# ningyu1991/InclusiveGAN

Measured on AMD Instinct MI355X. Metric: training img/sec (whole node), CelebA 128x128 StyleGAN2+IMLE, higher is better.
Workload: dtype f32-equivalent (3x3 convs: 2-piece fp16 split, operands to <= 1 ulp of fp32, scales per pixel / per channel: no per-tensor window; fp32 sums)

## Files before the change

### inclusivegan_amd/csrc/conv2d_mfma.hip

```cpp
#include "igan_common.h"
#include <cmath>
#include <cstdlib>
#include <type_traits>

namespace {

typedef float f32x16 __attribute__((ext_vector_type(16)));

constexpr int BK = 32;
#ifndef IGAN_SPLIT
#define IGAN_SPLIT 8
#endif
constexpr int LDK = BK + 4;

struct ConvArgs {
    const float* x;
    const float* w;
    float* y;
    float* out;
    const float* in_scale;
    const float* out_scale;
    int N, H, W, Cin;
    int OH, OW, Cout;
    int KH, KW;
// ... 2483 lines not shown
            const f16x8 b0 = __builtin_bit_cast(f16x8, tr8(S, fB[0], fB[1]));
            const f16x8 b1 = __builtin_bit_cast(f16x8, tr8(S + 4096, fB[0], fB[1]));
#pragma unroll
            for (int tm = 0; tm < TM; tm++) {
                a0[tm] = __builtin_bit_cast(f16x8, tr8(S, fA[tm][0], fA[tm][1]));
                a1[tm] = __builtin_bit_cast(f16x8, tr8(S + 4096, fA[tm][0], fA[tm][1]));
            }
            dma_prep(nst);
            f32x16 t;
            __builtin_amdgcn_sched_barrier(0);
            t = __builtin_amdgcn_mfma_f32_32x32x16_f16(a0[0], b0, zero, 0, 0, 0);
            u[0] = __builtin_amdgcn_mfma_f32_32x32x16_f16(a0[0], b1, u[0], 0, 0, 0);
            u[1] = __builtin_amdgcn_mfma_f32_32x32x16_f16(a0[1], b1, u[1], 0, 0, 0);
            __builtin_amdgcn_sched_barrier(0);
            dma_piece(0); dma_piece(1);
            acc[0] += t;
            __builtin_amdgcn_sched_barrier(0);
            t = __builtin_amdgcn_mfma_f32_32x32x16_f16(a0[1], b0, zero, 0, 0, 0);
            u[0] = __builtin_amdgcn_mfma_f32_32x32x16_f16(a1[0], b0, u[0], 0, 0, 0);
            u[1] = __builtin_amdgcn_mfma_f32_32x32x16_f16(a1[1], b0, u[1], 0, 0, 0);
            acc[1] += t;
            st = (st + 1 == P_NSTAGE) ? 0 : st + 1;
        }
        const float* xinv = reinterpret_cast<const float*>(reinterpret_cast<const unsigned char*>(a.xp) + (size_t)a.N * a.H * a.W * a.Cin * 4);
        const float* dyinv = reinterpret_cast<const float*>(reinterpret_cast<const unsigned char*>(a.dyp) + (size_t)a.N * a.OH * a.OW * a.Cout * 4);
        const int co_ = n0 + wn * 32 + l31;
        const float inv_b = (co_ < a.Cout) ? dyinv[co_] : 0.0f;
#pragma unroll
        for (int tm = 0; tm < TM; tm++)
#pragma unroll
            for (int q = 0; q < 4; q++) {
                const int ci = m0 + wm * 64 + tm * 32 + 8 * q + 4 * h;
                const float4 ia = (ci < a.Cin) ? *reinterpret_cast<const float4*>(xinv + ci) : f4zero();
                acc[tm][4 * q + 0] = ((acc[tm][4 * q + 0] + u[tm][4 * q + 0] * (1.0f / 2048.0f)) * ia.x) * inv_b;
                acc[tm][4 * q + 1] = ((acc[tm][4 * q + 1] + u[tm][4 * q + 1] * (1.0f / 2048.0f)) * ia.y) * inv_b;
                acc[tm][4 * q + 2] = ((acc[tm][4 * q + 2] + u[tm][4 * q + 2] * (1.0f / 2048.0f)) * ia.z) * inv_b;
                acc[tm][4 * q + 3] = ((acc[tm][4 * q + 3] + u[tm][4 * q + 3] * (1.0f / 2048.0f)) * ia.w) * inv_b;
            }
    } else
    for (int c = c_begin; c < c_end; c++) {
        asm volatile("s_waitcnt vmcnt(3)\n\ts_barrier" ::: "memory");
        const int nst = st >= 1 ? st - 1 : P_NSTAGE - 1;
        const unsigned char* S = smem + st * STAGE;
        bf16x8 af[TM][3], bfr[3];
#pragma unroll
        for (int q = 0; q < 3; q++) {
            bfr[q] = tr8(S + q * 4096, fB[0], fB[1]);
#pragma unroll
            for (int tm = 0; tm < TM; tm++) af[tm][q] = tr8(S + q * 4096, fA[tm][0], fA[tm][1]);
        }
        dma_prep(nst);
        f32x16 t[TM];
        __builtin_amdgcn_sched_barrier(0);
#pragma unroll
        for (int tm = 0; tm < TM; tm++) t[tm] = __builtin_amdgcn_mfma_f32_32x32x16_bf16(af[tm][0], bfr[0], zero, 0, 0, 0);
        int g = 0;
#pragma unroll
        for (int o = 1; o < 3; o++)
#pragma unroll
            for (int i = 0; i <= o; i++) {
                if (g == 2) { __builtin_amdgcn_sched_barrier(0); dma_piece(0); dma_piece(1); dma_piece(2); __builtin_amdgcn_sched_barrier(0); }
#pragma unroll
                for (int tm = 0; tm < TM; tm++) t[tm] = __builtin_amdgcn_mfma_f32_32x32x16_bf16(af[tm][i], bfr[o - i], t[tm], 0, 0, 0);
                ++g;
            }
#pragma unroll
        for (int tm = 0; tm < TM; tm++) acc[tm] += t[tm];
        st = (st + 1 == P_NSTAGE) ? 0 : st + 1;
    }
    drain_lds_dma();
    const size_t wsize = (size_t)a.KH * a.KW * a.Cin * a.Cout;
    float* out = a.out + (a.splits > 1 ? (size_t)split * wsize : (size_t)0) + (size_t)tap * a.Cin * a.Cout;
    const float alpha = (a.splits == 1) ? a.alpha : 1.0f;
    const int co = n0 + wn * 32 + l31;
#pragma unroll
    for (int tm = 0; tm < TM; tm++)
#pragma unroll
        for (int r = 0; r < 16; r++) {
            const int ci = m0 + wm * 64 + tm * 32 + (r & 3) + 8 * (r >> 2) + 4 * h;
            if (ci < a.Cin && co < a.Cout) out[(size_t)ci * a.Cout + co] = acc[tm][r] * alpha;
        }
}

__global__ __launch_bounds__(256) void plain_reduce_kernel(const float* ws, float* y, int total, int splits, float alpha) {
    for (int i = blockIdx.x * blockDim.x + threadIdx.x; i < total; i += gridDim.x * blockDim.x) {
        float s0 = 0.f, s1 = 0.f, s2 = 0.f, s3 = 0.f;
        int k = 0;
        for (; k + 4 <= splits; k += 4) {
            const float a0 = ws[(size_t)k * total + i], a1 = ws[(size_t)(k + 1) * total + i];
            const float a2 = ws[(size_t)(k + 2) * total + i], a3 = ws[(size_t)(k + 3) * total + i];
            s0 += a0; s1 += a1; s2 += a2; s3 += a3;
        }
        for (; k < splits; k++) s0 += ws[(size_t)k * total + i];
        y[i] = ((s0 + s1) + (s2 + s3)) * alpha;
    }
}

struct FwdTile { int BM, BN; };

FwdTile pick_fwd_tile(int Mmax, int Cout) {
    FwdTile t;
    t.BN = (Cout > 64) ? 128 : (Cout > 32 ? 64 : 32);
    t.BM = (Mmax <= 32 && t.BN == 128) ? 32 : 128;
    return t;
}

int fwd_geometry_check(const igan_conv2d_params* p) {
    IGAN_REQUIRE(p->x && p->w && p->y, "conv2d: null buffer");
    IGAN_REQUIRE(p->N >= 1 && p->H >= 1 && p->W >= 1 && p->Cin >= 1, "conv2d: input dims must be positive");
    IGAN_REQUIRE(p->OH >= 1 && p->OW >= 1 && p->Cout >= 1, "conv2d: output dims must be positive");
    IGAN_REQUIRE(p->KH >= 1 && p->KW >= 1, "conv2d: kernel must be at least 1x1");
    IGAN_REQUIRE(p->stride >= 1 && p->up >= 1, "conv2d: stride and up must be at least 1");
    IGAN_REQUIRE(p->stride == 1 || p->up == 1, "conv2d: at most one of stride, up may exceed 1");
    if (!(p->up == 1 || p->up == 2)) return igan::fail(IGAN_ERR_UNSUPPORTED, "conv2d: up must be 1 or 2 (got %d)", p->up);
    IGAN_REQUIRE((long long)p->N * p->H * p->W * p->Cin * 4 <= 0x7FFFFFF0LL, "conv2d: input too large (2 GiB per operand)");
    IGAN_REQUIRE((long long)p->N * p->OH * p->OW * p->Cout <= INT32_MAX, "conv2d: output too large");
    IGAN_REQUIRE((long long)p->KH * p->KW * p->Cin * p->Cout * 4 <= 0x7FFFFFF0LL, "conv2d: filter too large (2 GiB per operand)");
    IGAN_REQUIRE(p->act >= 0 && p->act <= 3, "conv2d: fused epilogue act must be 0 (none), 1 linear, 2 relu or 3 lrelu");
    IGAN_REQUIRE(p->act == 0 || p->act_gain > 0.0f, "conv2d: fused epilogue gain must be positive");
    IGAN_REQUIRE(p->noise == nullptr || (p->act != 0 && p->noise_strength != nullptr), "conv2d: noise needs the fused epilogue (act != 0) and a strength scalar");
    return IGAN_OK;
}

bool eight_waves(const char* env) {
    const char* v = getenv(env);
    return !(v && atoi(v) == 0);
}

bool is_small_dense(const igan_conv2d_params* p) {
    return p->H == 1 && p->W == 1 && p->OH == 1 && p->OW == 1 && p->KH == 1 && p->KW == 1 && p->stride == 1 && p->up == 1 &&
           p->pad_y == 0 && p->pad_x == 0 && !p->in_scale && !p->out_scale && p->act == 0 &&
           igan::dense_small_ok(p->N, p->Cin, p->Cout, p->x, p->w, p->w_transposed != 0);
}
bool is_small_dense_wgrad(const igan_conv2d_wgrad_params* p) {
    return p->H == 1 && p->W == 1 && p->OH == 1 && p->OW == 1 && p->KH == 1 && p->KW == 1 && p->stride == 1 && p->up == 1 &&
           p->pad_y == 0 && p->pad_x == 0 && !p->in_scale && !p->out_scale &&
           igan::dense_small_wgrad_ok(p->N, p->Cout, p->dy, p->dw);
}

void fwd_counts(const igan_conv2d_params* p, int& Mmax, int& chunks_max, int& nclass) {
    const int up = p->up;
    nclass = up * up;
    const int QH = (p->OH + up - 1) / up, QW = (p->OW + up - 1) / up;
    Mmax = p->N * QH * QW;
    const int cpt = (p->Cin + BK - 1) / BK;
    chunks_max = ((p->KH + up - 1) / up) * ((p->KW + up - 1) / up) * cpt;
}

template <int BM, int BN, int WM, int WN, bool WT, bool VEC>
void launch_fwd2(hipStream_t stream, const ConvArgs& a, dim3 grid) {
    if (a.in_scale) hipLaunchKernelGGL((conv_fwd_kernel<BM, BN, WM, WN, WT, VEC, true>), grid, dim3(WM * WN * 64), 0, stream, a);
    else hipLaunchKernelGGL((conv_fwd_kernel<BM, BN, WM, WN, WT, VEC, false>), grid, dim3(WM * WN * 64), 0, stream, a);
}

template <int BM, int BN, int WM, int WN>
void launch_fwd(hipStream_t stream, const ConvArgs& a, dim3 grid, bool wt, bool vec) {
    if (wt) {
        if (vec) launch_fwd2<BM, BN, WM, WN, true, true>(stream, a, grid);
        else launch_fwd2<BM, BN, WM, WN, true, false>(stream, a, grid);
    } else {
        if (vec) launch_fwd2<BM, BN, WM, WN, false, true>(stream, a, grid);
        else launch_fwd2<BM, BN, WM, WN, false, false>(stream, a, grid);
    }
}

}
// ... 10 lines not shown
        (void)hipGetLastError();
        cus = n;
    }
    return cus;
}

struct TileList { int nx, ny, T, rem; };
TileList tile_list(const igan_conv2d_params* p, const FwdTile& t, int Mmax, int nclass) {
    TileList l;
    l.nx = igan::ceil_div(Mmax, t.BM);
    l.ny = igan::ceil_div(p->Cout, t.BN);
    l.T = l.nx * l.ny * nclass;
    l.rem = l.T % device_cus();
    return l;
}


bool use_dma_kernel(const igan_conv2d_params* p, const FwdTile& t, bool walk) {
    static const bool dma = !(getenv("IGAN_CONV_DMA") && atoi(getenv("IGAN_CONV_DMA")) == 0);
    if (!dma || t.BM != 128 || t.BN != 128 || !walk || !eight_waves("IGAN_CONV_8WAVE")) return false;
    if ((long long)p->N * p->OH * p->OW >= (1LL << 24)) return false;
    if (p->in_scale) {
        const int up = p->up;
        for (int c = 0; c < up * up; c++) {
            const int qh = (p->OH - c / up + up - 1) / up, qw = (p->OW - c % up + up - 1) / up;
            if (qh <= 0 || qw <= 0) continue;
            const int samples = 127 / (qh * qw) + 2;
            if ((long long)std::min(samples, p->N) * p->Cin > 2048) return false;
        }
    }
    return true;
}

bool walk_ok(const igan_conv2d_params* p) {
    static const bool walk = !(getenv("IGAN_CONV_WALK") && atoi(getenv("IGAN_CONV_WALK")) == 0);
    const bool wt = p->w_transposed != 0;
    const bool vecA = (p->Cin % 4 == 0) && (((uintptr_t)p->x & 15) == 0);
    const bool vecS = (p->Cin % 4 == 0) && (((uintptr_t)p->in_scale & 15) == 0);
    const bool vecB = ((wt ? p->Cin : p->Cout) % 4 == 0) && (((uintptr_t)p->w & 15) == 0);
    return walk && vecA && vecB && (p->in_scale == nullptr || vecS) && (p->Cin % BK == 0);
}

int planes_mode() {
    static const int mode = [] { const char* v = getenv("IGAN_CONV_PLANES"); const int m = v ? atoi(v) : 2; return m == 0 ? 0 : (m == 1 ? 1 : 2); }();
    return mode;
}
bool planes_enabled() { return planes_mode() != 0; }

int ilog2(int v) { int l = 0; while ((1 << l) < v) ++l; return l; }
bool pow2(int v) { return v > 0 && (v & (v - 1)) == 0; }

void launch_piece_image(hipStream_t stream, const float* x, const float* scale, unsigned short* out, int P_, int HW, int C) {
    const int cpp = C / PK, total = P_ * cpp;
    hipLaunchKernelGGL(to_planes_kernel, dim3(igan::ceil_div(total, 256)), dim3(256), 0, stream, x, scale, out, total, cpp, C, HW);
}
void launch_row_image(hipStream_t stream, const float* x, const float* scale, unsigned short* out, int P_, int HW, int C, float* colmax) {
    const int cpp = C / PK, total = P_ * cpp;
    float* rowinv = reinterpret_cast<float*>(reinterpret_cast<unsigned char*>(out) + (size_t)P_ * C * 4);
    const int nchunks = igan::ceil_div(total, 256);
    const int grid = colmax ? std::min(nchunks, H_COLBLOCKS) : nchunks;
    hipLaunchKernelGGL(rows_f16_kernel, dim3(grid), dim3(256), 0, stream, x, scale, out, rowinv, colmax, total, cpp, ilog2(cpp), C, HW);
}
void launch_colmax_only(hipStream_t stream, const float* x, const float* scale, float* colmax, int P_, int HW, int C) {
    const int C4 = C / 4, ppi = 256 / C4;
    const int blocks = std::min(H_COLBLOCKS, igan::ceil_div(P_, ppi));
    hipLaunchKernelGGL(cols_amax_kernel, dim3(blocks), dim3(256), 0, stream, x, scale, colmax + 4, P_, C4, ilog2(C4), HW, colmax);
}
void launch_col_image(hipStream_t stream, const float* x, const float* scale, unsigned short* out, int P_, int HW, int C, const float* colmax) {
    const int cpp = C / PK, total = P_ * cpp, C4 = C / 4;
    float* inv = reinterpret_cast<float*>(reinterpret_cast<unsigned char*>(out) + (size_t)P_ * C * 4);
    float* sc = inv + C;
    float* partial = sc + C;
    const int ppi = 256 / C4;
    const int blocks = std::min(H_COLBLOCKS, igan::ceil_div(P_, ppi));
    if (colmax == nullptr) {
        hipLaunchKernelGGL(cols_amax_kernel, dim3(blocks), dim3(256), 0, stream, x, scale, partial, P_, C4, ilog2(C4), HW, (float*)nullptr);
        hipLaunchKernelGGL(cols_finalize_kernel, dim3(igan::ceil_div(C, 8)), dim3(256), 0, stream, (const float*)partial, inv, sc, blocks, C, (const float*)nullptr);
    } else
        hipLaunchKernelGGL(cols_finalize_kernel, dim3(igan::ceil_div(C, 8)), dim3(256), 0, stream, colmax + 4, inv, sc, 0, C, colmax);
    hipLaunchKernelGGL(cols_f16_kernel, dim3(igan::ceil_div(total, 256)), dim3(256), 0, stream, x, scale, out, (const float*)sc, total, cpp, C, HW);
}
bool f16_tap_outer() { static const int v = getenv("IGAN_F16_TAP_OUTER") ? atoi(getenv("IGAN_F16_TAP_OUTER")) : 1; return v != 0; }
bool f16_w4() { static const int v = getenv("IGAN_F16_W4") ? atoi(getenv("IGAN_F16_W4")) : 1; return v != 0; }
void launch_filter_image(hipStream_t stream, const float* w, unsigned short* wp, bool wt, int taps, int KW_, int Nn, int K) {
    const int wtotal = taps * Nn * (K / PK);
    if (planes_mode() == 2) {
        float* inv = reinterpret_cast<float*>(reinterpret_cast<unsigned char*>(wp) + (size_t)taps * Nn * K * 4);
        float* partial = inv + Nn;
        if (wt) {
            hipLaunchKernelGGL((filter_amax_kernel<true>), dim3(igan::ceil_div(taps * Nn, 4)), dim3(256), 0, stream, w, partial, taps, Nn, K);
            hipLaunchKernelGGL((filter_planes_f16_kernel<true>), dim3(igan::ceil_div(wtotal, 256)), dim3(256), 0, stream, w, wp, inv, (const float*)partial, taps, taps, KW_, Nn, K);
        } else {
            hipLaunchKernelGGL((filter_amax_kernel<false>), dim3(taps * H_KSK, igan::ceil_div(Nn, 64)), dim3(256), 0, stream, w, partial, taps, Nn, K);
            hipLaunchKernelGGL((filter_planes_f16_kernel<false>), dim3(igan::ceil_div(wtotal, 256)), dim3(256), 0, stream, w, wp, inv, (const float*)partial, taps * H_KSK, taps, KW_, Nn, K);
        }
    } else {
        if (wt) hipLaunchKernelGGL((filter_planes_kernel<true>), dim3(igan::ceil_div(wtotal, 256)), dim3(256), 0, stream, w, wp, taps, KW_, Nn, K);
        else hipLaunchKernelGGL((filter_planes_kernel<false>), dim3(igan::ceil_div(wtotal, 256)), dim3(256), 0, stream, w, wp, taps, KW_, Nn, K);
    }
}

bool planes_shape_ok(const igan_conv2d_params* p, const FwdTile& t, int Mmax) {
    if (!planes_enabled() || t.BM != 128 || t.BN != 128 || p->Cin % BK != 0) return false;
    static const int min_rows = getenv("IGAN_PLANES_MIN_ROWS") ? atoi(getenv("IGAN_PLANES_MIN_ROWS")) : 1024;
    if (p->KH * p->KW == 1 || (long long)p->KH * p->KW * p->Cin < 1152 || Mmax < min_rows) return false;
    if ((long long)p->N * p->OH * p->OW >= (1LL << 24)) return false;
    if ((long long)p->N * p->H * p->W * p->Cin * 6 >= 0x7FFFFF00LL || (long long)p->KH * p->KW * p->Cin * p->Cout * 6 >= 0x7FFFFF00LL) return false;
    if (planes_mode() == 2 && (!pow2(p->Cin / PK) || p->Cin / PK > 64 || p->KH * p->KW > 9 || p->Cout % 4 != 0)) return false;
#ifdef IGAN_DIAGNOSTIC
    {
        static const int only_cin = getenv("IGAN_PLANES_ONLY_CIN") ? atoi(getenv("IGAN_PLANES_ONLY_CIN")) : 0;
        static const int no_act = getenv("IGAN_PLANES_NO_ACT") ? atoi(getenv("IGAN_PLANES_NO_ACT")) : 0;
        static const int no_scale = getenv("IGAN_PLANES_NO_SCALE") ? atoi(getenv("IGAN_PLANES_NO_SCALE")) : 0;
        static const int kind = getenv("IGAN_PLANES_KIND") ? atoi(getenv("IGAN_PLANES_KIND")) : 0;
        static const int wt = getenv("IGAN_PLANES_WT") ? atoi(getenv("IGAN_PLANES_WT")) : 0;
        if (only_cin && p->Cin != only_cin) return false;
        if ((no_act == 1 && p->act != 0) || (no_act == 2 && p->act == 0)) return false;
        if ((no_scale == 1 && p->in_scale != nullptr) || (no_scale == 2 && p->in_scale == nullptr)) return false;
        if ((kind == 1 && (p->stride != 1 || p->up != 1)) || (kind == 2 && p->stride != 2) || (kind == 3 && p->up != 2)) return false;
        if ((wt == 1 && p->w_transposed) || (wt == 2 && !p->w_transposed)) return false;
    }
#endif
    return true;
}
bool use_planes_kernel(const igan_conv2d_params* p, const FwdTile& t, int Mmax) {
    if (!planes_shape_ok(p, t, Mmax) || (((uintptr_t)p->x | (uintptr_t)p->w | (uintptr_t)p->in_scale | (uintptr_t)p->x_pieces) & 15) != 0) return false;
    if (planes_mode() == 2 && (((uintptr_t)p->y | (uintptr_t)p->out_scale | (uintptr_t)p->bias) & 15) != 0) return false;
    return true;
}
size_t planes_x_floats(const igan_conv2d_params* p) {
    if (planes_mode() == 2) return rows_part_bytes((size_t)p->N * p->H * p->W, (size_t)p->Cin) / 4;
    return (size_t)p->N * p->H * p->W * p->Cin * 6 / 4;
}
size_t planes_w_floats(const igan_conv2d_params* p) {
    if (planes_mode() == 2) return filter_part_bytes((size_t)p->KH * p->KW, (size_t)p->Cout, (size_t)p->Cin) / 4;
    return (size_t)p->KH * p->KW * p->Cin * p->Cout * 6 / 4;
}

}

static unsigned long long* g_conv_diag = nullptr;
extern "C" void igan_debug_set_conv_diag(unsigned long long* p) { g_conv_diag = p; }

static int conv2d_plan_tiles(const igan_conv2d_params* p, int* splits, int* sliced_tiles, size_t* workspace_floats);

extern "C" int igan_conv2d_plan(const igan_conv2d_params* p, int* splits, int* sliced_tiles, size_t* workspace_floats) {
    IGAN_REQUIRE(p && splits && sliced_tiles && workspace_floats, "conv2d_plan: null argument");
    if (int rc = fwd_geometry_check(p)) return rc;
    *splits = 1;
    *sliced_tiles = 0;
    *workspace_floats = 0;
    if (is_small_dense(p) || igan::thin_conv_kind(p)) return IGAN_OK;
    if (int rc = conv2d_plan_tiles(p, splits, sliced_tiles, workspace_floats)) return rc;
    int Mmax, chunks_max, nclass;
    fwd_counts(p, Mmax, chunks_max, nclass);
    if (planes_shape_ok(p, pick_fwd_tile(Mmax, p->Cout), Mmax))
        *workspace_floats += planes_x_floats(p) + planes_w_floats(p);
    return IGAN_OK;
}

static int conv2d_plan_tiles(const igan_conv2d_params* p, int* splits, int* sliced_tiles, size_t* workspace_floats) {
    int Mmax, chunks_max, nclass;
    fwd_counts(p, Mmax, chunks_max, nclass);
    const FwdTile t = pick_fwd_tile(Mmax, p->Cout);
    const TileList l = tile_list(p, t, Mmax, nclass);
    {
// ... 248 lines not shown
    WgTile t;
    t.BM = (Cin > 32) ? 128 : 32;
    t.BN = (Cout > 32) ? 128 : 32;
    if (t.BM == 32 && t.BN == 32) t.BN = 128;
    return t;
}

int wgrad_splits(const igan_conv2d_wgrad_params* p) {
    const WgTile t = pick_wg_tile(p->Cin, p->Cout);
    const long long tiles = (long long)igan::ceil_div(p->Cin, t.BM) * igan::ceil_div(p->Cout, t.BN) * p->KH * p->KW;
    const int up = p->up;
    const long long kpix = (long long)p->N * ((p->OH + up - 1) / up) * ((p->OW + up - 1) / up);
    const int chunks = (int)((kpix + BK - 1) / BK);
    const int max_by_work = std::max(1, chunks / 4);
    int s;
    if (tiles >= 512) s = 1;
    else {
        s = (int)(512 / tiles);
        if (s > max_by_work) s = max_by_work;
        else if (chunks / s > 96 && 1024 / tiles <= max_by_work) s = (int)(1024 / tiles);
    }
    s = std::min(s, 256);
    return std::max(s, 1);
}

int wgrad_min_rows() {
    static const int v = getenv("IGAN_WGRAD_PLANES_MIN_ROWS") ? atoi(getenv("IGAN_WGRAD_PLANES_MIN_ROWS")) : 1024;
    return v;
}
bool wgrad_planes_shape_ok(const igan_conv2d_wgrad_params* p) {
    static const bool wg = !(getenv("IGAN_WGRAD_PLANES") && atoi(getenv("IGAN_WGRAD_PLANES")) == 0);
    if (!planes_enabled() || !wg || p->KH * p->KW == 1 || p->Cin < 128 || p->Cout < 128 || p->Cin % 32 != 0 || p->Cout % 32 != 0) return false;
#ifdef IGAN_DIAGNOSTIC
    {
        static const int only_cin = getenv("IGAN_WGRAD_PLANES_CIN") ? atoi(getenv("IGAN_WGRAD_PLANES_CIN")) : 0;
        static const char* kind = getenv("IGAN_WGRAD_PLANES_KIND");
        if (only_cin && p->Cin != only_cin) return false;
        if (kind && kind[0] == 'p' && (p->stride != 1 || p->up != 1)) return false;
        if (kind && kind[0] == 's' && p->stride != 2) return false;
        if (kind && kind[0] == 'u' && p->up != 2) return false;
    }
#endif
    if ((long long)p->N * p->OH * p->OW < wgrad_min_rows() * (long long)p->up * p->up) return false;
    if ((long long)p->N * p->H * p->W * p->Cin * 6 >= 0x7FFFFF00LL || (long long)p->N * p->OH * p->OW * p->Cout * 6 >= 0x7FFFFF00LL) return false;
    if (planes_mode() == 2 && (!pow2(p->Cin) || !pow2(p->Cout) || p->Cin > 1024 || p->Cout > 1024)) return false;
    return true;
}
size_t wgrad_planes_x_floats(const igan_conv2d_wgrad_params* p) {
    if (planes_mode() == 2) return cols_part_bytes((size_t)p->N * p->H * p->W, (size_t)p->Cin) / 4;
    return (size_t)p->N * p->H * p->W * p->Cin * 6 / 4;
}
size_t wgrad_planes_dy_floats(const igan_conv2d_wgrad_params* p) {
    if (planes_mode() == 2) return cols_part_bytes((size_t)p->N * p->OH * p->OW, (size_t)p->Cout) / 4;
    return (size_t)p->N * p->OH * p->OW * p->Cout * 6 / 4;
}

}

extern "C" int igan_conv2d_wgrad_plan(const igan_conv2d_wgrad_params* p, int* splits, size_t* workspace_floats) {
    IGAN_REQUIRE(p && splits && workspace_floats, "conv2d_wgrad_plan: null argument");
    if (int rc = wgrad_geometry_check(p)) return rc;
    if (is_small_dense_wgrad(p)) { *splits = 1; *workspace_floats = 0; return IGAN_OK; }
    if (const int kind = igan::thin_wgrad_kind(p)) {
        *splits = 2;
        *workspace_floats = igan::thin_wgrad_workspace(p, kind);
        return IGAN_OK;
    }
    const int s = wgrad_splits(p);
    *splits = s;
    *workspace_floats = (s > 1) ? (size_t)s * p->KH * p->KW * p->Cin * p->Cout : 0;
    if (wgrad_planes_shape_ok(p))
        *workspace_floats += wgrad_planes_x_floats(p) + wgrad_planes_dy_floats(p);
    return IGAN_OK;
}

extern "C" int igan_conv2d_wgrad_kernel_name(const igan_conv2d_wgrad_params* p, char* buf, int buflen) {
    using namespace igan;
    IGAN_REQUIRE(p && buf && buflen > 0, "conv2d_wgrad_kernel_name: null argument");
    if (int rc = wgrad_geometry_check(p)) return rc;
    const char* name = "conv_wgrad_kernel";
    if (is_small_dense_wgrad(p)) name = "dense_small_wgrad_kernel";
    else if (thin_wgrad_kind(p)) name = "thin_wgrad_kernel";
    else if (wgrad_planes_shape_ok(p) && (((uintptr_t)p->x | (uintptr_t)p->dy | (uintptr_t)p->in_scale | (uintptr_t)p->out_scale | (uintptr_t)p->x_pieces | (uintptr_t)p->dy_pieces) & 15) == 0)
        name = "conv_wgrad_planes_kernel";
    snprintf(buf, (size_t)buflen, "%s", name);
    return IGAN_OK;
}

extern "C" int igan_conv2d_wgrad(igan_stream_t stream_, const igan_conv2d_wgrad_params* p) {
    using namespace igan;
    hipStream_t stream = (hipStream_t)stream_;
    IGAN_REQUIRE(p != nullptr, "conv2d_wgrad: null params");
    if (int rc = wgrad_geometry_check(p)) return rc;
    if (is_small_dense_wgrad(p)) {
        dense_small_wgrad(stream, p->x, p->dy, p->dw, p->N, p->Cin, p->Cout, p->alpha);
        IGAN_LAUNCH_CHECK("conv2d_wgrad dense launch");
        return IGAN_OK;
    }
    if (const int kind = thin_wgrad_kind(p)) {
        if (p->workspace && p->workspace_floats >= thin_wgrad_workspace(p, kind) && (((uintptr_t)p->workspace) & 15) == 0) {
            thin_wgrad(stream, p, kind);
            IGAN_LAUNCH_CHECK("conv2d_wgrad thin-channel launch");
            return IGAN_OK;
        }
    }
    const int splits = std::max(1, p->splits);
    const size_t wsize = (size_t)p->KH * p->KW * p->Cin * p->Cout;
    if (splits > 1) {
        IGAN_REQUIRE(p->workspace != nullptr, "conv2d_wgrad: splits > 1 needs a workspace");
        IGAN_REQUIRE(p->workspace_floats >= (size_t)splits * wsize, "conv2d_wgrad: workspace too small");
    }
    if (p->x_colmax != nullptr) IGAN_REQUIRE(igan_colmax_floats(p->N, p->H * p->W, p->Cin) != 0 && (((uintptr_t)p->x_colmax) & 15) == 0, "conv2d_wgrad: x_colmax is not a buffer igan_colmax_floats() sized for this x");
    if (p->dy_colmax != nullptr) IGAN_REQUIRE(igan_colmax_floats(p->N, p->OH * p->OW, p->Cout) != 0 && (((uintptr_t)p->dy_colmax) & 15) == 0, "conv2d_wgrad: dy_colmax is not a buffer igan_colmax_floats() sized for this dy");
    WgradArgs a;
    a.x = p->x; a.dy = p->dy;
    a.out = (splits > 1) ? p->workspace : p->dw;
    a.in_scale = p->in_scale; a.out_scale = p->out_scale;
    a.N = p->N; a.H = p->H; a.W = p->W; a.Cin = p->Cin;
    a.OH = p->OH; a.OW = p->OW; a.Cout = p->Cout;
    a.KH = p->KH; a.KW = p->KW;
    a.stride = p->stride; a.up_shift = (p->up == 2) ? 1 : 0;
    a.pad_y = p->pad_y; a.pad_x = p->pad_x;
    a.splits = splits;
    a.vecA = (p->Cin % 4 == 0) && (((uintptr_t)p->x & 15) == 0);
    a.vecB = (p->Cout % 4 == 0) && (((uintptr_t)p->dy & 15) == 0);
    a.vecSA = (p->Cin % 4 == 0) && (((uintptr_t)p->in_scale & 15) == 0);
    a.vecSB = (p->Cout % 4 == 0) && (((uintptr_t)p->out_scale & 15) == 0);

    a.vecY = (p->Cout % 2 == 0) && (((uintptr_t)a.out & 7) == 0);
    a.alpha = p->alpha;
    {
        static const bool remap = !(getenv("IGAN_XCD_REMAP") && atoi(getenv("IGAN_XCD_REMAP")) == 0);
        a.xcd_remap = remap ? 1 : 0;
    }

    const WgTile t = pick_wg_tile(p->Cin, p->Cout);
    dim3 grid(ceil_div(p->Cin, t.BM), ceil_div(p->Cout, t.BN), p->KH * p->KW * splits);
    a.xp = nullptr; a.dyp = nullptr;
    const size_t partial_floats = (splits > 1) ? (size_t)splits * wsize : 0;
    if (wgrad_planes_shape_ok(p) && p->workspace != nullptr && (((uintptr_t)p->workspace | (uintptr_t)p->x | (uintptr_t)p->dy | (uintptr_t)p->in_scale | (uintptr_t)p->out_scale | (uintptr_t)p->x_pieces | (uintptr_t)p->dy_pieces) & 15) == 0 &&
        p->workspace_floats >= partial_floats + wgrad_planes_x_floats(p) + wgrad_planes_dy_floats(p)) {
        IGAN_REQUIRE((p->x_pieces == nullptr && p->dy_pieces == nullptr) || planes_mode() == 1, "conv2d_wgrad: the two-piece fp16 form writes its own images (one scale per channel): x_pieces / dy_pieces must be NULL");
        IGAN_REQUIRE(p->x_pieces == nullptr || p->x_pieces_bytes == wgrad_planes_x_floats(p) * 4, "conv2d_wgrad: x_pieces is not the image of this x (x_pieces_bytes != N*H*W*Cin*6)");
        IGAN_REQUIRE(p->dy_pieces == nullptr || p->dy_pieces_bytes == wgrad_planes_dy_floats(p) * 4, "conv2d_wgrad: dy_pieces is not the image of this dy (dy_pieces_bytes != N*OH*OW*Cout*6)");
        const unsigned short* xp = reinterpret_cast<const unsigned short*>(p->x_pieces);
        const unsigned short* dyp = reinterpret_cast<const unsigned short*>(p->dy_pieces);
        if (xp == nullptr) {
            unsigned short* own = reinterpret_cast<unsigned short*>(p->workspace + partial_floats);
            if (planes_mode() == 2) launch_col_image(stream, p->x, p->in_scale, own, p->N * p->H * p->W, p->H * p->W, p->Cin, p->x_colmax);
            else launch_piece_image(stream, p->x, p->in_scale, own, p->N * p->H * p->W, p->H * p->W, p->Cin);
            xp = own;
        }
        if (dyp == nullptr) {
            unsigned short* own = reinterpret_cast<unsigned short*>(p->workspace + partial_floats + wgrad_planes_x_floats(p));
            if (planes_mode() == 2) launch_col_image(stream, p->dy, p->out_scale, own, p->N * p->OH * p->OW, p->OH * p->OW, p->Cout, p->dy_colmax);
            else launch_piece_image(stream, p->dy, p->out_scale, own, p->N * p->OH * p->OW, p->OH * p->OW, p->Cout);
            dyp = own;
        }
        a.xp = xp; a.dyp = dyp;
        if (planes_mode() == 2) hipLaunchKernelGGL((conv_wgrad_planes_kernel<2>), grid, dim3(512), 0, stream, a);
        else hipLaunchKernelGGL((conv_wgrad_planes_kernel<3>), grid, dim3(512), 0, stream, a);
        IGAN_LAUNCH_CHECK("conv2d_wgrad (piece form) launch");
        if (splits > 1) {
            const int total = (int)wsize;
            const int rg = std::min(ceil_div(total, 256), 2048);
            hipLaunchKernelGGL(plain_reduce_kernel, dim3(rg), dim3(256), 0, stream, (const float*)p->workspace, p->dw, total, splits, p->alpha);
            IGAN_LAUNCH_CHECK("conv2d_wgrad reduce launch");
        }
        return IGAN_OK;
    }
    const bool vec = a.vecA && a.vecB && (a.in_scale == nullptr || a.vecSA) && (a.out_scale == nullptr || a.vecSB);
    const int scm = (a.in_scale && a.out_scale) ? 1 : ((a.in_scale || a.out_scale) ? 2 : 0);
    const bool long_axis = (long long)p->OH * p->OW >= 128LL * 128LL;
    if (t.BM == 128 && t.BN == 128 && eight_waves("IGAN_WGRAD_8WAVE") && !long_axis && scm == 0) launch_wgrad<128, 128, 2, 4>(stream, a, grid, vec, scm);
    else if (t.BM == 128 && t.BN == 128) launch_wgrad<128, 128, 2, 2>(stream, a, grid, vec, scm);
    else if (t.BM == 128 && t.BN == 32) launch_wgrad<128, 32, 4, 1>(stream, a, grid, vec, scm);
    else launch_wgrad<32, 128, 1, 4>(stream, a, grid, vec, scm);
    IGAN_LAUNCH_CHECK("conv2d_wgrad launch");
    if (splits > 1) {
        const int total = (int)wsize;
        const int rg = std::min(ceil_div(total, 256), 2048);
        hipLaunchKernelGGL(plain_reduce_kernel, dim3(rg), dim3(256), 0, stream, (const float*)p->workspace, p->dw, total, splits, p->alpha);
        IGAN_LAUNCH_CHECK("conv2d_wgrad reduce launch");
    }
    return IGAN_OK;
}

static int f16_window_read(unsigned long long (&v)[4], int reset) {
    using namespace igan;
    if (hipMemcpyFromSymbol(&v[0], HIP_SYMBOL(g_f16_below_window), 8) != hipSuccess || hipMemcpyFromSymbol(&v[1], HIP_SYMBOL(g_f16_imaged), 8) != hipSuccess ||
        hipMemcpyFromSymbol(&v[2], HIP_SYMBOL(g_f16_below_window_cols), 8) != hipSuccess || hipMemcpyFromSymbol(&v[3], HIP_SYMBOL(g_f16_imaged_cols), 8) != hipSuccess) return IGAN_ERR_HIP;
    if (reset) {
        const unsigned long long z = 0ull;
        if (hipMemcpyToSymbol(HIP_SYMBOL(g_f16_below_window), &z, 8) != hipSuccess || hipMemcpyToSymbol(HIP_SYMBOL(g_f16_imaged), &z, 8) != hipSuccess ||
            hipMemcpyToSymbol(HIP_SYMBOL(g_f16_below_window_cols), &z, 8) != hipSuccess || hipMemcpyToSymbol(HIP_SYMBOL(g_f16_imaged_cols), &z, 8) != hipSuccess) return IGAN_ERR_HIP;
    }
    return IGAN_OK;
}
extern "C" int igan_debug_f16_window(unsigned long long* below, unsigned long long* imaged, int reset) {
    unsigned long long v[4] = {0ull, 0ull, 0ull, 0ull};
    if (int rc = f16_window_read(v, reset)) return rc;
    if (below) *below = v[0] + v[2];
    if (imaged) *imaged = v[1] + v[3];
    return IGAN_OK;
}
extern "C" int igan_debug_f16_window_by_kind(unsigned long long* out4, int reset) {
    using namespace igan;
    IGAN_REQUIRE(out4 != nullptr, "debug_f16_window_by_kind: null argument");
    unsigned long long v[4] = {0ull, 0ull, 0ull, 0ull};
    if (int rc = f16_window_read(v, reset)) return rc;
    for (int i = 0; i < 4; i++) out4[i] = v[i];
    return IGAN_OK;
}

extern "C" int igan_conv_piece_form(void) { return planes_mode(); }

extern "C" size_t igan_colmax_floats(int N, int HW, int C) {
    using namespace igan;
    if (planes_mode() != 2 || N < 1 || HW < 1 || C < 16 || C > 1024 || (C & (C - 1)) != 0) return 0;
    if ((long long)N * HW < wgrad_min_rows()) return 0;
    return 4 + (size_t)H_COLBLOCKS * C;
}

extern "C" size_t igan_filter_image_bytes(int KH, int KW, int Cin, int Cout) {
    using namespace igan;
    if (!planes_enabled() || KH < 1 || KW < 1 || Cin < 1 || Cout < 1 || KH * KW == 1 || Cin % BK != 0 || (long long)KH * KW * Cin < 1152) return 0;
    if ((long long)KH * KW * Cin * Cout * 6 >= 0x7FFFFF00LL) return 0;
    if (planes_mode() == 2) {
        if (!pow2(Cin / PK) || Cin / PK > 64 || KH * KW > 9 || Cout % 4 != 0) return 0;
        return filter_part_bytes((size_t)KH * KW, (size_t)Cout, (size_t)Cin);
    }
    return (size_t)KH * KW * Cin * Cout * 6;
}

extern "C" int igan_filter_image(igan_stream_t stream_, const float* w, void* out, int KH, int KW, int Cin, int Cout, int w_transposed) {
    using namespace igan;
    IGAN_REQUIRE(w != nullptr && out != nullptr, "filter_image: null buffer");
    IGAN_REQUIRE(igan_filter_image_bytes(KH, KW, Cin, Cout) != 0, "filter_image: igan_filter_image_bytes() says this process / filter takes none");
    IGAN_REQUIRE(((((uintptr_t)w) | ((uintptr_t)out)) & 15) == 0, "filter_image: w and out must be 16-byte aligned");
    launch_filter_image((hipStream_t)stream_, w, reinterpret_cast<unsigned short*>(out), w_transposed != 0, KH * KW, KW, Cout, Cin);
    IGAN_LAUNCH_CHECK("filter_image launch");
    return IGAN_OK;
}
// ... 23 lines not shown
```

Before: 356.5.

## Add 4-wave pipelined two-piece fp16 wgrad planes kernel with transpose LDS reads

Adds a new 256-thread weight-gradient kernel for the two-piece fp16 planes mode and makes it the default path. It uses a 3-stage LDS DMA pipeline, ds_read_b64_tr_b16 transposed fragment reads, explicit waitcnt/barrier and sched_barrier interleaving of MFMAs with DMA issue, and 2x2 32x32 tiles per wave that accumulate hi and lo pieces separately. The aim is to replace the 512-thread generic planes kernel and hide global-to-LDS latency behind MFMA work. In exchange it adds hand-written asm scheduling that is complex and fragile, and it relies on a grid shape that must match the old launch.

After: 359.0, median of 6. About the same (+0.7%).

```diff
diff --git a/inclusivegan_amd/csrc/conv2d_mfma.hip b/inclusivegan_amd/csrc/conv2d_mfma.hip
--- a/inclusivegan_amd/csrc/conv2d_mfma.hip
+++ b/inclusivegan_amd/csrc/conv2d_mfma.hip
@@ -2589,6 +2589,229 @@
         }
 }
 
+template <int OFF>
+__device__ __forceinline__ f16x8 tr8_asm(unsigned v0, unsigned v1) {
+    s16x4 lo, hi;
+    asm volatile("ds_read_b64_tr_b16 %0, %1 offset:%2" : "=v"(lo) : "v"(v0), "n"(OFF));
+    asm volatile("ds_read_b64_tr_b16 %0, %1 offset:%2" : "=v"(hi) : "v"(v1), "n"(OFF));
+    typedef __attribute__((ext_vector_type(8))) short s16x8;
+    return __builtin_bit_cast(f16x8, (s16x8)__builtin_shufflevector(lo, hi, 0, 1, 2, 3, 4, 5, 6, 7));
+}
+__global__ __launch_bounds__(256, 2) void conv_wgrad_planes_w4_kernel(WgradArgs a) {
+    constexpr int NS = 3;
+    constexpr int IMG = 2 * 4096, STAGE = 2 * IMG;
+    constexpr unsigned PB = 64u;
+    __shared__ __attribute__((aligned(1024))) unsigned char smem[NS * STAGE];
+    const int tid = threadIdx.x;
+    const int lane = tid & 63, wave = __builtin_amdgcn_readfirstlane(tid >> 6);
+    const int l31 = lane & 31, h = lane >> 5;
+    const int wm = wave >> 1, wn = wave & 1;
+    const int up = 1 << a.up_shift;
+    int bx = blockIdx.x, by = blockIdx.y, bz = blockIdx.z;
+    int tap = bz / a.splits, split = bz - tap * a.splits;
+    if (a.xcd_remap) {
+        const int gx = gridDim.x, gy = gridDim.y, taps = a.KH * a.KW;
+        const int lin = remap_xcd(bx + gx * (by + gy * bz), gx * gy * (int)gridDim.z);
+        tap = lin % taps;
+        int rest = lin / taps;
+        bx = rest % gx; rest /= gx;
+        by = rest % gy;
+        split = rest / gy;
+    }
+    const int ky = tap / a.KW, kx = tap - ky * a.KW;
+    const int py = (a.pad_y - ky) & (up - 1);
+    const int px = (a.pad_x - kx) & (up - 1);
+    const int QH = (a.OH - py + up - 1) >> a.up_shift;
+    const int QW = (a.OW - px + up - 1) >> a.up_shift;
+    const int Kpix = (QH > 0 && QW > 0) ? a.N * QH * QW : 0;
+    const int chunks = (Kpix + PK - 1) / PK;
+    const int c_begin = (int)(((long long)split * chunks) / a.splits);
+    const int c_end = (int)(((long long)(split + 1) * chunks) / a.splits);
+    const bool any = c_begin < c_end;
+    const int m0 = bx * 128, n0 = by * 128;
+    const int s_in = (up == 1) ? a.stride : 1;
+    const int cy = (up == 1) ? ky - a.pad_y : (py + ky - a.pad_y) >> 1;
+    const int cx = (up == 1) ? kx - a.pad_x : (px + kx - a.pad_x) >> 1;
+
+    const int drow = 4 * wave + (lane >> 4);
+    const int dch = (lane & 15) ^ (((drow & 3) << 2) | ((drow >> 2) & 3));
+    const unsigned rowA = (unsigned)a.Cin * 4u, rowB = (unsigned)a.Cout * 4u;
+    const bool chA = m0 + 8 * dch < a.Cin, chB = n0 + 8 * dch < a.Cout;
+    const unsigned constA = (unsigned)((m0 >> 4) + (dch >> 1)) * PB + (unsigned)(dch & 1) * 16u;
+    const unsigned constB = (unsigned)((n0 >> 4) + (dch >> 1)) * PB + (unsigned)(dch & 1) * 16u;
+    const int dQW = max(QW, 1), dQH = max(QH, 1);
+    const int st_b = PK % dQW, st_a = PK / dQW, st_a2 = st_a % dQH, st_a1 = st_a / dQH;
+    int kp = c_begin * PK + drow, wqy = 0, wqx = 0;
+    unsigned linA, linB;
+    {
+        const int wn_ = kp / (dQH * dQW);
+        const int r = kp - wn_ * (dQH * dQW);
+        wqy = r / dQW; wqx = r - wqy * dQW;
+        const int iy0 = wqy * s_in + cy, ix0 = wqx * s_in + cx;
+        linA = (unsigned)((wn_ * a.H + iy0) * a.W + ix0) * rowA + constA;
+        const int oy0 = (wqy << a.up_shift) + py, ox0 = (wqx << a.up_shift) + px;
+        linB = (unsigned)((wn_ * a.OH + oy0) * a.OW + ox0) * rowB + constB;
+    }
+    const unsigned dA0 = (unsigned)((st_a1 * a.H + s_in * st_a2) * a.W + s_in * st_b) * rowA;
+    const unsigned dA1 = (unsigned)(s_in * a.W - s_in * QW) * rowA;
+    const unsigned dA2 = (unsigned)((a.H - s_in * QH) * a.W) * rowA;
+    const unsigned dB0 = (unsigned)((st_a1 * a.OH + up * st_a2) * a.OW + up * st_b) * rowB;
+    const unsigned dB1 = (unsigned)(up * a.OW - up * QW) * rowB;
+    const unsigned dB2 = (unsigned)((a.OH - up * QH) * a.OW) * rowB;
+    const unsigned xbytes = (unsigned)a.N * a.H * a.W * a.Cin * 4u, dybytes = (unsigned)a.N * a.OH * a.OW * a.Cout * 4u;
+    const u32x4 wx = raw_rsrc_words(a.xp, xbytes), wdy = raw_rsrc_words(a.dyp, dybytes);
+    typedef __attribute__((address_space(3))) void lds_void;
+    const unsigned lds0 = (unsigned)(unsigned long long)(lds_void*)smem;
+    unsigned offA = OOB, offB = OOB;
+    auto dma_prep = [&]() {
+        const int iy = __mul24(wqy, s_in) + cy, ix = __mul24(wqx, s_in) + cx;
+        const bool live = kp < Kpix;
+        const bool okA = live & chA & ((unsigned)iy < (unsigned)a.H) & ((unsigned)ix < (unsigned)a.W);
+        offA = okA ? linA : OOB;
+        offB = (live & chB) ? linB : OOB;
+        kp += PK;
+        wqx += st_b;
+        const bool c1 = wqx >= QW;
+        wqx -= c1 ? QW : 0;
+        wqy += st_a2 + (c1 ? 1 : 0);
+        const bool c2 = wqy >= QH;
+        wqy -= c2 ? QH : 0;
+        linA += dA0 + (c1 ? dA1 : 0u) + (c2 ? dA2 : 0u);
+        linB += dB0 + (c1 ? dB1 : 0u) + (c2 ? dB2 : 0u);
+    };
+    auto dma_pair = [&](int stage, int which) {
+        const unsigned D = lds0 + (unsigned)(stage * STAGE + wave * 1024);
+        if (which == 0) { lds_dma16_asm<0>(wx, D, offA); lds_dma16_asm<32>(wx, D + 4096, offA); }
+        else { lds_dma16_asm<0>(wdy, D + IMG, offB); lds_dma16_asm<32>(wdy, D + IMG + 4096, offB); }
+    };
+
+    const int tg = lane >> 4, tq = (lane >> 2) & 3, tp = lane & 3;
+    unsigned fA[2][2], fB[2][2];
+#pragma unroll
+    for (int hf = 0; hf < 2; hf++) {
+        const int row = 8 * (tg >> 1) + 4 * hf + tq;
+        const int xr = ((row & 3) << 2) | ((row >> 2) & 3);
+#pragma unroll
+        for (int t = 0; t < 2; t++) {
+            const int chunk = wm * 8 + t * 4 + 2 * (tg & 1) + (tp >> 1);
+            fA[t][hf] = lds0 + (unsigned)(256 * row + 16 * (chunk ^ xr) + 8 * (tp & 1));
+            const int chunkb = (wn * 2 + t) * 4 + 2 * (tg & 1) + (tp >> 1);
+            fB[t][hf] = lds0 + (unsigned)(IMG + 256 * row + 16 * (chunkb ^ xr) + 8 * (tp & 1));
+        }
+    }
+    struct Frag { f16x8 a0[2], a1[2], b0[2], b1[2]; };
+    auto read_frags = [&](Frag& f, int stage) {
+        const unsigned so = (unsigned)(stage * STAGE);
+        f.b0[0] = tr8_asm<0>(fB[0][0] + so, fB[0][1] + so);
+        f.a0[0] = tr8_asm<0>(fA[0][0] + so, fA[0][1] + so);
+        f.b1[0] = tr8_asm<4096>(fB[0][0] + so, fB[0][1] + so);
+        f.b1[1] = tr8_asm<4096>(fB[1][0] + so, fB[1][1] + so);
+        f.a0[1] = tr8_asm<0>(fA[1][0] + so, fA[1][1] + so);
+        f.b0[1] = tr8_asm<0>(fB[1][0] + so, fB[1][1] + so);
+        f.a1[0] = tr8_asm<4096>(fA[0][0] + so, fA[0][1] + so);
+        f.a1[1] = tr8_asm<4096>(fA[1][0] + so, fA[1][1] + so);
+    };
+
+    f32x16 acc[2][2], u[2][2];
+#pragma unroll
+    for (int i = 0; i < 2; i++)
+#pragma unroll
+        for (int j = 0; j < 2; j++)
+#pragma unroll
+            for (int r = 0; r < 16; r++) { acc[i][j][r] = 0.0f; u[i][j][r] = 0.0f; }
+    const f32x16 zero = {0.f, 0.f, 0.f, 0.f, 0.f, 0.f, 0.f, 0.f, 0.f, 0.f, 0.f, 0.f, 0.f, 0.f, 0.f, 0.f};
+    int st = 0;
+    Frag F0, F1;
+    auto step = [&](Frag& cur, Frag& nxt, auto tail) {
+        constexpr bool TAIL = decltype(tail)::value;
+        int st1 = st;
+        if constexpr (TAIL) {
+            asm volatile("s_waitcnt lgkmcnt(0)"
+                         : "+v"(cur.a0[0]), "+v"(cur.a0[1]), "+v"(cur.a1[0]), "+v"(cur.a1[1]), "+v"(cur.b0[0]), "+v"(cur.b0[1]), "+v"(cur.b1[0]), "+v"(cur.b1[1]) :: "memory");
+        } else {
+            asm volatile("s_waitcnt vmcnt(4) lgkmcnt(0)\n\ts_barrier"
+                         : "+v"(cur.a0[0]), "+v"(cur.a0[1]), "+v"(cur.a1[0]), "+v"(cur.a1[1]), "+v"(cur.b0[0]), "+v"(cur.b0[1]), "+v"(cur.b1[0]), "+v"(cur.b1[1]) :: "memory");
+            st1 = (st + 1 == NS) ? 0 : st + 1;
+            read_frags(nxt, st1);
+            dma_prep();
+        }
+        f32x16 tA, tB;
+        const auto SB = [] { __builtin_amdgcn_sched_barrier(0); };
+        SB();
+        tA = __builtin_amdgcn_mfma_f32_32x32x16_f16(cur.a0[0], cur.b0[0], zero, 0, 0, 0);
+        SB();
+        u[0][0] = __builtin_amdgcn_mfma_f32_32x32x16_f16(cur.a0[0], cur.b1[0], u[0][0], 0, 0, 0);
+        u[0][1] = __builtin_amdgcn_mfma_f32_32x32x16_f16(cur.a0[0], cur.b1[1], u[0][1], 0, 0, 0);
+        SB();
+        if constexpr (!TAIL) dma_pair(st, 0);
+        SB();
+        tB = __builtin_amdgcn_mfma_f32_32x32x16_f16(cur.a0[0], cur.b0[1], zero, 0, 0, 0);
+        SB();
+        acc[0][0] += tA;
+        SB();
+        u[1][0] = __builtin_amdgcn_mfma_f32_32x32x16_f16(cur.a0[1], cur.b1[0], u[1][0], 0, 0, 0);
+        u[1][1] = __builtin_amdgcn_mfma_f32_32x32x16_f16(cur.a0[1], cur.b1[1], u[1][1], 0, 0, 0);
+        SB();
+        if constexpr (!TAIL) dma_pair(st, 1);
+        SB();
+        tA = __builtin_amdgcn_mfma_f32_32x32x16_f16(cur.a0[1], cur.b0[0], zero, 0, 0, 0);
+        SB();
+        acc[0][1] += tB;
+        SB();
+        u[0][0] = __builtin_amdgcn_mfma_f32_32x32x16_f16(cur.a1[0], cur.b0[0], u[0][0], 0, 0, 0);
+        u[0][1] = __builtin_amdgcn_mfma_f32_32x32x16_f16(cur.a1[0], cur.b0[1], u[0][1], 0, 0, 0);
+        SB();
+        tB = __builtin_amdgcn_mfma_f32_32x32x16_f16(cur.a0[1], cur.b0[1], zero, 0, 0, 0);
+        SB();
+        acc[1][0] += tA;
+        SB();
+        u[1][0] = __builtin_amdgcn_mfma_f32_32x32x16_f16(cur.a1[1], cur.b0[0], u[1][0], 0, 0, 0);
+        u[1][1] = __builtin_amdgcn_mfma_f32_32x32x16_f16(cur.a1[1], cur.b0[1], u[1][1], 0, 0, 0);
+        SB();
+        acc[1][1] += tB;
+        st = st1;
+    };
+    if (any) {
+#pragma unroll
+        for (int j = 0; j < NS; j++) { dma_prep(); dma_pair(j, 0); dma_pair(j, 1); }
+        asm volatile("s_waitcnt vmcnt(8)\n\ts_barrier" ::: "memory");
+        read_frags(F0, 0);
+        int c = c_begin;
+        for (; c + 1 < c_end; c += 2) { step(F0, F1, std::false_type()); step(F1, F0, std::false_type()); }
+        if (c < c_end) step(F0, F1, std::true_type());
+        else
+            asm volatile("s_waitcnt lgkmcnt(0)"
+                         :: "v"(F0.a0[0]), "v"(F0.a0[1]), "v"(F0.a1[0]), "v"(F0.a1[1]), "v"(F0.b0[0]), "v"(F0.b0[1]), "v"(F0.b1[0]), "v"(F0.b1[1]) : "memory");
+    }
+    drain_lds_dma();
+    const float* xinv = reinterpret_cast<const float*>(reinterpret_cast<const unsigned char*>(a.xp) + (size_t)a.N * a.H * a.W * a.Cin * 4);
+    const float* dyinv = reinterpret_cast<const float*>(reinterpret_cast<const unsigned char*>(a.dyp) + (size_t)a.N * a.OH * a.OW * a.Cout * 4);
+    const size_t wsize = (size_t)a.KH * a.KW * a.Cin * a.Cout;
+    float* out = a.out + (a.splits > 1 ? (size_t)split * wsize : (size_t)0) + (size_t)tap * a.Cin * a.Cout;
+    const float alpha = (a.splits == 1) ? a.alpha : 1.0f;
+#pragma unroll
+    for (int tn = 0; tn < 2; tn++) {
+        const int co = n0 + wn * 64 + tn * 32 + l31;
+        const float inv_b = (co < a.Cout) ? dyinv[co] : 0.0f;
+#pragma unroll
+        for (int tm = 0; tm < 2; tm++)
+#pragma unroll
+            for (int q = 0; q < 4; q++) {
+                const int ci = m0 + wm * 64 + tm * 32 + 8 * q + 4 * h;
+                const float4 ia = (ci < a.Cin) ? *reinterpret_cast<const float4*>(xinv + ci) : f4zero();
+                const float v[4] = {((acc[tm][tn][4 * q + 0] + u[tm][tn][4 * q + 0] * (1.0f / 2048.0f)) * ia.x) * inv_b,
+                                    ((acc[tm][tn][4 * q + 1] + u[tm][tn][4 * q + 1] * (1.0f / 2048.0f)) * ia.y) * inv_b,
+                                    ((acc[tm][tn][4 * q + 2] + u[tm][tn][4 * q + 2] * (1.0f / 2048.0f)) * ia.z) * inv_b,
+                                    ((acc[tm][tn][4 * q + 3] + u[tm][tn][4 * q + 3] * (1.0f / 2048.0f)) * ia.w) * inv_b};
+                if (co < a.Cout) {
+#pragma unroll
+                    for (int i = 0; i < 4; i++)
+                        if (ci < a.Cin) out[(size_t)(ci + i) * a.Cout + co] = v[i] * alpha;
+                }
+            }
+    }
+}
+
 __global__ __launch_bounds__(256) void plain_reduce_kernel(const float* ws, float* y, int total, int splits, float alpha) {
     for (int i = blockIdx.x * blockDim.x + threadIdx.x; i < total; i += gridDim.x * blockDim.x) {
         float s0 = 0.f, s1 = 0.f, s2 = 0.f, s3 = 0.f;
@@ -2765,6 +2988,7 @@
 }
 bool f16_tap_outer() { static const int v = getenv("IGAN_F16_TAP_OUTER") ? atoi(getenv("IGAN_F16_TAP_OUTER")) : 1; return v != 0; }
 bool f16_w4() { static const int v = getenv("IGAN_F16_W4") ? atoi(getenv("IGAN_F16_W4")) : 1; return v != 0; }
+bool wgrad_w4() { static const int v = getenv("IGAN_WGRAD_W4") ? atoi(getenv("IGAN_WGRAD_W4")) : 1; return v != 0; }
 void launch_filter_image(hipStream_t stream, const float* w, unsigned short* wp, bool wt, int taps, int KW_, int Nn, int K) {
     const int wtotal = taps * Nn * (K / PK);
     if (planes_mode() == 2) {
@@ -3179,7 +3403,7 @@
     if (is_small_dense_wgrad(p)) name = "dense_small_wgrad_kernel";
     else if (thin_wgrad_kind(p)) name = "thin_wgrad_kernel";
     else if (wgrad_planes_shape_ok(p) && (((uintptr_t)p->x | (uintptr_t)p->dy | (uintptr_t)p->in_scale | (uintptr_t)p->out_scale | (uintptr_t)p->x_pieces | (uintptr_t)p->dy_pieces) & 15) == 0)
-        name = "conv_wgrad_planes_kernel";
+        name = (planes_mode() == 2 && wgrad_w4()) ? "conv_wgrad_planes_w4_kernel" : "conv_wgrad_planes_kernel";
     snprintf(buf, (size_t)buflen, "%s", name);
     return IGAN_OK;
 }
@@ -3255,7 +3479,8 @@
             dyp = own;
         }
         a.xp = xp; a.dyp = dyp;
-        if (planes_mode() == 2) hipLaunchKernelGGL((conv_wgrad_planes_kernel<2>), grid, dim3(512), 0, stream, a);
+        if (planes_mode() == 2 && wgrad_w4()) hipLaunchKernelGGL(conv_wgrad_planes_w4_kernel, grid, dim3(256), 0, stream, a);
+        else if (planes_mode() == 2) hipLaunchKernelGGL((conv_wgrad_planes_kernel<2>), grid, dim3(512), 0, stream, a);
         else hipLaunchKernelGGL((conv_wgrad_planes_kernel<3>), grid, dim3(512), 0, stream, a);
         IGAN_LAUNCH_CHECK("conv2d_wgrad (piece form) launch");
         if (splits > 1) {
```
